# opensensor/thingino-accel

Measured on AMD Instinct MI355X. Metric: images/sec yolov5s_int8 640x640 batch256, higher is better.
Workload: dtype int8

## Files before the change

thingino-accel_amd/csrc/hip/conv_i8.hip:

```cpp
#include "conv_i8_common.hpp"

#ifndef I8M_ABL
#define I8M_ABL 0
#endif
template <int BPX, int BN, int STAGES, int KS = 1, int NW = 4>
__global__ __launch_bounds__(NW * 64) void conv_i8_mfma(const mhip_conv_i8_t p, const long total_pix, const int k64,
                                                         const int8_t *__restrict__ zeros, const unsigned noc,
                                                         const unsigned nblk, const int lg_inc, const unsigned kw_magic,
                                                         const fastdiv_t dhw, const fastdiv_t dow, const int bufmode,
                                                         const unsigned in_bytes) {
    ANAT_BEGIN();
    const bool POW2 = lg_inc >= 0;
    const bool masked = p.kh * p.kw <= 32;
    constexpr int SLICE = (BPX + BN) * BK;
    constexpr int STAGE = KS * SLICE;
    constexpr int NWN = BN == 128 ? 2 : 1;
    constexpr int NWM = NW / NWN;
    constexpr int WPX = BPX / NWM / 16;
    constexpr int WOC = BN / NWN / 16;
    constexpr int XROWS = BPX / NW;
    constexpr int XI = XROWS / 16;
    constexpr int LW = (BN / 16 + NW - 1) / NW;
    constexpr int L = XI + LW;
    static_assert(XI >= 1 && XROWS % 16 == 0, "every wave fetches whole 16-row pieces of the pixel tile");
    extern __shared__ __attribute__((aligned(16))) int8_t dynlds[];
    uint8_t *slut = (uint8_t *)dynlds;
    lds_base_must_be_zero(dynlds);
    long *rowoff = (long *)(dynlds + LUTB);
    int8_t *lds = dynlds + BPX * 8 + LUTB;

    const int tid = threadIdx.x, lane = tid & 63;
    const int wv = __builtin_amdgcn_readfirstlane(tid >> 6);
    const unsigned id = xcd_remap(blockIdx.x, nblk);
    const long pix0 = (long)(id / noc) * BPX;
    const int oc0 = (int)(id % noc) * BN;
    const int hw = p.out_h * p.out_w;

    const int wm = wv % NWM, wn = wv / NWM;
    const int pxw = wm * (WPX * 16), ocw = wn * (WOC * 16);
    v4i acc[WOC][WPX];
    init_acc<WPX, WOC>(p, acc, oc0 + ocw);
    if (p.lut2) { if (tid < 128) ((uint32_t *)slut)[tid] = ((const uint32_t *)p.lut2)[tid]; }
    else if (p.lut && tid < 64) ((uint32_t *)slut)[tid] = ((const uint32_t *)p.lut)[tid];
    fill_rowoff<BPX>(p, rowoff, [=](int row) { long q = pix0 + row; return q < total_pix ? q : -1L; }, (unsigned)hw, dhw);

    const int schunk = (lane & 3) ^ (((lane >> 4) & 1) << 1);
    const int8_t *xwin[XI];
    unsigned tapmask[XI];
    int iy0[XI], ix0[XI];
#pragma unroll
    for (int j = 0; j < XI; j++) {
        const long pix = pix0 + wv * XROWS + j * 16 + (lane >> 2);
        const bool valid = pix < total_pix;
        const unsigned f = valid ? fdiv((unsigned)pix, dhw) : 0u;
        const unsigned rem = valid ? (unsigned)pix - f * (unsigned)hw : 0u;
        const int oy = (int)fdiv(rem, dow), ox = (int)(rem - (unsigned)oy * (unsigned)p.out_w);
        iy0[j] = valid ? oy * p.stride_h - p.pad_top : -(1 << 28);
        ix0[j] = ox * p.stride_w - p.pad_left;
        xwin[j] = p.in + (size_t)f * p.in_stride + ((long)iy0[j] * p.in_w + ix0[j]) * p.in_c;
        unsigned m = 0;
        if (masked) {
            const int kx_lo = ix0[j] < 0 ? -ix0[j] : 0, kx_hi = p.in_w - ix0[j] < p.kw ? p.in_w - ix0[j] : p.kw;
            const unsigned colbits = kx_hi > kx_lo ? ((kx_hi >= 32 ? ~0u : (1u << kx_hi) - 1u) & ~((1u << kx_lo) - 1u)) : 0u;
            for (int r = 0; r < p.kh; r++) {
                const int iy = iy0[j] + r;
                if (iy >= 0 && iy < p.in_h) m |= colbits << (r * p.kw);
            }
        }
        tapmask[j] = m;
    }
    const int8_t *wsrc[LW];
    int wq[LW];
#pragma unroll
    for (int j = 0; j < LW; j++) {
        wq[j] = BN / 16 >= NW ? wv * LW + j : (wv % (BN / 16));
        wsrc[j] = p.w + (size_t)(oc0 + wq[j] * 16 + (lane >> 2)) * k64 + schunk * 16;
    }
    const __amdgpu_buffer_rsrc_t xrs = __builtin_amdgcn_make_buffer_rsrc((void *)p.in, 0, (int)in_bytes, 0x00020000);
    const __amdgpu_buffer_rsrc_t wrs = __builtin_amdgcn_make_buffer_rsrc((void *)p.w, 0, p.oc_pad * k64, 0x00020000);
    int xvoff[XI], wvoff[LW];
    if (bufmode) {
#pragma unroll
        for (int j = 0; j < XI; j++) xvoff[j] = (int)(xwin[j] - p.in) + schunk * 16;
#pragma unroll
        for (int j = 0; j < LW; j++) wvoff[j] = (oc0 + wq[j] * 16 + (lane >> 2)) * k64 + schunk * 16;
    }
    int ky = 0, kx = 0, rc = schunk * 16;
    if (!POW2) {
        while (rc >= p.in_c) { rc -= p.in_c; kx++; }
        while (kx >= p.kw) { kx -= p.kw; ky++; }
    }
    const int taps = p.kh * p.kw;

    const int nks = k64 / BK;
    auto issue = [&](int ks, int stage) {
        int8_t *sb = lds + stage * STAGE + (KS > 1 ? (ks % KS) * SLICE : 0);
        if (bufmode) {
            const int utap = (ks * BK) >> lg_inc, urc = (ks * BK) & ((1 << lg_inc) - 1);
            const int uky = (int)(((unsigned)utap * kw_magic) >> 16), ukx = utap - uky * p.kw;
            const int ukoff = (uky * p.in_w + ukx) * p.in_c + urc;
            const bool uvalid = utap < taps;
#pragma unroll
            for (int j = 0; j < XI; j++) {
                const bool ok = uvalid & (((tapmask[j] >> utap) & 1u) != 0u);
                if (!(I8M_ABL & 8)) blds16(xrs, ok ? xvoff[j] + ukoff : -1, 0, sb + (wv * XROWS + j * 16) * BK);
            }
#pragma unroll
            for (int j = 0; j < LW; j++)
                if (!(I8M_ABL & 8)) blds16(wrs, wvoff[j], ks * BK, sb + BPX * BK + wq[j] * 16 * BK);
            return;
        }
        bool kvalid;
        if (POW2) {
            const unsigned pos = (unsigned)(ks * BK + schunk * 16);
            const unsigned tap = pos >> lg_inc;
            rc = (int)(pos & ((1u << lg_inc) - 1u));
            ky = (int)((tap * kw_magic) >> 16);
            kx = (int)tap - ky * p.kw;
            kvalid = (int)tap < taps;
        } else {
            kvalid = ky < p.kh;
        }
        const long koff = ((long)ky * p.in_w + kx) * p.in_c + rc;
        const int tap = ky * p.kw + kx;
#pragma unroll
        for (int j = 0; j < XI; j++) {
            bool ok;
            if (masked) {
                ok = kvalid & ((tapmask[j] >> tap) & 1u);
            } else {
                const int iy = iy0[j] + ky, ix = ix0[j] + kx;
                ok = kvalid & (iy >= 0) & (iy < p.in_h) & (ix >= 0) & (ix < p.in_w);
            }
            const int8_t *src = ok ? xwin[j] + koff : zeros;
            glds16(src, sb + (wv * XROWS + j * 16) * BK);
        }
#pragma unroll
        for (int j = 0; j < LW; j++) glds16(wsrc[j] + ks * BK, sb + BPX * BK + wq[j] * 16 * BK);
        if (!POW2) {
            rc += BK;
            while (rc >= p.in_c) { rc -= p.in_c; kx++; }
            while (kx >= p.kw) { kx -= p.kw; ky++; }
        }
    };

    const int nst = I8M_ABL & 2 ? 0 : nks / KS;
#pragma unroll
    for (int s = 0; s < STAGES - 1; s++)
        if (s < nst)
#pragma unroll
            for (int u = 0; u < KS; u++) issue(s * KS + u, s);

    const int frow = lane & 15, fchunk = lane >> 4;
    int stage = 0, nstage = STAGES - 1;
    ANAT_NOW(1);
    for (int st = 0; st < nst; st++) {
        const int ahead = nst - 1 - st;
        if (STAGES >= 4 && ahead >= 2) wait_vmcnt<2 * L * KS>();
        else if (STAGES >= 3 && ahead >= 1) wait_vmcnt<L * KS>();
        else wait_vmcnt<0>();
        __builtin_amdgcn_s_barrier();
        asm volatile("" ::: "memory");
#pragma unroll
        for (int u = 0; u < KS; u++) {
            const int8_t *xs = lds + stage * STAGE + u * SLICE, *ws = xs + BPX * BK;
            v4i xb[WPX], wa[WOC];
#pragma unroll
            for (int t = 0; t < WPX; t++) xb[t] = *(const v4i *)(xs + lds_off(pxw + t * 16 + frow, fchunk));
#pragma unroll
            for (int s = 0; s < WOC; s++) wa[s] = *(const v4i *)(ws + lds_off(ocw + s * 16 + frow, fchunk));
            if (u == 0 && st + STAGES - 1 < nst)
#pragma unroll
                for (int v = 0; v < KS; v++) issue((st + STAGES - 1) * KS + v, nstage);
#pragma unroll
            for (int s = 0; s < WOC; s++)
#pragma unroll
                for (int t = 0; t < WPX; t++) {
                    if (I8M_ABL & 4) asm volatile("" ::"v"(wa[s]), "v"(xb[t]));
                    else acc[s][t] = __builtin_amdgcn_mfma_i32_16x16x64_i8(wa[s], xb[t], acc[s][t], 0, 0, 0);
                }
        }
        stage = stage + 1 == STAGES ? 0 : stage + 1;
        nstage = nstage + 1 == STAGES ? 0 : nstage + 1;
    }
    ANAT_NOW(2);
    __syncthreads();
    if (I8M_ABL & 1) {
        int fold = 0;
#pragma unroll
        for (int s = 0; s < WOC; s++)
#pragma unroll
            for (int t = 0; t < WPX; t++) fold ^= acc[s][t][0] ^ acc[s][t][1] ^ acc[s][t][2] ^ acc[s][t][3];
        if (fold == 0x12345678) p.out[0] = 1;
        return;
    }
    epilogue<BPX, BN, WPX, WOC, true>(p, acc, lds, slut, rowoff, oc0, pxw, ocw, hw);
    ANAT_END(p);
}

__device__ __forceinline__ int lds_off128(int row, int chunk8) { return row * 128 + ((chunk8 ^ ((row >> 1) & 7)) << 4); }
template <int BPX, int BN, int NW>
__global__ __launch_bounds__(NW * 64) void conv_i8_r128(const mhip_conv_i8_t p, const long total_pix, const int k128,
                                                         const unsigned noc, const unsigned nblk, const int lg_inc,
                                                         const unsigned kw_magic, const fastdiv_t dhw, const fastdiv_t dow,
                                                         const unsigned in_bytes) {
    constexpr int STAGE = (BPX + BN) * 128;
    constexpr int NWN = BN == 128 ? 2 : 1;
    constexpr int NWM = NW / NWN;
    constexpr int WPX = BPX / NWM / 16;
    constexpr int WOC = BN / NWN / 16;
    constexpr int XI = BPX / 8 / NW;
    constexpr int WI = BN / 8 / NW;
    static_assert(XI >= 1 && WI >= 1 && BPX % (8 * NW) == 0 && BN % (8 * NW) == 0, "whole 8-row pieces per wave");
    extern __shared__ __attribute__((aligned(16))) int8_t dynlds[];
    uint8_t *slut = (uint8_t *)dynlds;
    lds_base_must_be_zero(dynlds);
    long *rowoff = (long *)(dynlds + LUTB);
    int8_t *lds = dynlds + BPX * 8 + LUTB;

    const int tid = threadIdx.x, lane = tid & 63;
    const int wv = __builtin_amdgcn_readfirstlane(tid >> 6);
    const unsigned id = xcd_remap(blockIdx.x, nblk);
    const long pix0 = (long)(id / noc) * BPX;
    const int oc0 = (int)(id % noc) * BN;
    const int hw = p.out_h * p.out_w;
    const int wm = wv % NWM, wn = wv / NWM;
    const int pxw = wm * (WPX * 16), ocw = wn * (WOC * 16);
    v4i acc[WOC][WPX];
    init_acc<WPX, WOC>(p, acc, oc0 + ocw);
    if (p.lut2) { if (tid < 128) ((uint32_t *)slut)[tid] = ((const uint32_t *)p.lut2)[tid]; }
    else if (p.lut && tid < 64) ((uint32_t *)slut)[tid] = ((const uint32_t *)p.lut)[tid];
    fill_rowoff<BPX>(p, rowoff, [=](int row) { long q = pix0 + row; return q < total_pix ? q : -1L; }, (unsigned)hw, dhw);

    const int lrow = lane >> 3, lslot = lane & 7;
    int xvoff[XI];
    unsigned tapmask[XI];
#pragma unroll
    for (int j = 0; j < XI; j++) {
        const int trow = (wv * XI + j) * 8 + lrow;
        const long pix = pix0 + trow;
        const bool valid = pix < total_pix;
        const unsigned f = valid ? fdiv((unsigned)pix, dhw) : 0u;
        const unsigned rem = valid ? (unsigned)pix - f * (unsigned)hw : 0u;
        const int oy = (int)fdiv(rem, dow), ox = (int)(rem - (unsigned)oy * (unsigned)p.out_w);
        const int iy0 = oy * p.stride_h - p.pad_top, ix0 = ox * p.stride_w - p.pad_left;
        const int chunk = lslot ^ ((trow >> 1) & 7);
        xvoff[j] = (int)(f * (unsigned)p.in_stride) + (iy0 * p.in_w + ix0) * p.in_c + chunk * 16;
        const int kx_lo = ix0 < 0 ? -ix0 : 0, kx_hi = p.in_w - ix0 < p.kw ? p.in_w - ix0 : p.kw;
        const unsigned colbits = kx_hi > kx_lo ? ((kx_hi >= 32 ? ~0u : (1u << kx_hi) - 1u) & ~((1u << kx_lo) - 1u)) : 0u;
        unsigned m = 0;
        for (int r = 0; r < p.kh; r++) {
            const int iy = iy0 + r;
            if (iy >= 0 && iy < p.in_h) m |= colbits << (r * p.kw);
        }
        tapmask[j] = valid ? m : 0u;
    }
    int wvoff[WI];
#pragma unroll
    for (int j = 0; j < WI; j++) {
        const int trow = (wv * WI + j) * 8 + lrow;
        wvoff[j] = (oc0 + trow) * k128 + (lslot ^ ((trow >> 1) & 7)) * 16;
    }
    const __amdgpu_buffer_rsrc_t xrs = __builtin_amdgcn_make_buffer_rsrc((void *)p.in, 0, (int)in_bytes, 0x00020000);
    const __amdgpu_buffer_rsrc_t wrs = __builtin_amdgcn_make_buffer_rsrc((void *)p.w, 0, p.oc_pad * k128, 0x00020000);
    const int taps = p.kh * p.kw;
    const int nst = k128 / 128;
    auto issue = [&](int st, int buf) {
        int8_t *sb = lds + buf * STAGE;
        const int utap = (st * 128) >> lg_inc, urc = (st * 128) & ((1 << lg_inc) - 1);
        const int uky = (int)(((unsigned)utap * kw_magic) >> 16), ukx = utap - uky * p.kw;
        const int ukoff = (uky * p.in_w + ukx) * p.in_c + urc;
        const bool uvalid = utap < taps;
#pragma unroll
        for (int j = 0; j < XI; j++) {
            const bool ok = uvalid & (((tapmask[j] >> utap) & 1u) != 0u);
            blds16(xrs, ok ? xvoff[j] + ukoff : -1, 0, sb + (wv * XI + j) * 1024);
// ... 416 lines not shown
    v4i acc[WOC][WPX];
    init_acc<WPX, WOC>(p, acc, oc0);

    load_global(0);
    store_lds(0);
    __syncthreads();
    const int frow = lane & 15, fchunk = lane >> 4;
    const int pxw = wv * 32;
    for (int ks = 0; ks < nks; ks++) {
        const int buf = ks & 1;
        if (ks + 1 < nks) load_global(ks + 1);
        v4i xb[WPX];
#pragma unroll
        for (int t = 0; t < WPX; t++) xb[t] = *(const v4i *)(lds + buf * STAGE + lds_off(pxw + t * 16 + frow, fchunk));
#pragma unroll
        for (int s = 0; s < WOC; s++) {
            v4i wa = *(const v4i *)(lds + buf * STAGE + BP * BK + lds_off(s * 16 + frow, fchunk));
#pragma unroll
            for (int t = 0; t < WPX; t++) acc[s][t] = __builtin_amdgcn_mfma_i32_16x16x64_i8(wa, xb[t], acc[s][t], 0, 0, 0);
        }
        if (ks + 1 < nks) store_lds(buf ^ 1);
        __syncthreads();
    }
    epilogue<BP, BN, WPX, WOC>(p, acc, lds, slut, rowoff, oc0, pxw, 0, hw);
}

extern "C" int mhip_conv_i8_oc_row(int oc, int oc_pad) {
    const int G = (oc_pad % 64 == 0) ? 64 : 32, NS = G / 16;
    const int g = oc / G, local = oc - g * G;
    const int q = local / (4 * NS), rem = local - q * 4 * NS, s = rem >> 2, r = rem & 3;
    return g * G + s * 16 + q * 4 + r;
}

extern "C" int mhip_conv_i8_is_safe(float cs) {
    return cs == cs && cs < 0.99f && cs > -0.99f;
}

extern "C" int mhip_conv_i8_lut2_ok(float cs) {
    if (!mhip_conv_i8_is_safe(cs)) return 0;
    const float a = cs < 0 ? -cs : cs;
    if (!(a >= 1e-6f)) return 0;
    const float quirk = 0.49999997f;
    const double a0 = (double)quirk / (double)a;
    for (int d = -3; d <= 3; d++) {
        const double c = (double)(long long)(a0 + 0.5) + d;
        if (c < 1.0 || c > 2147483647.0) continue;
        volatile float prod = (float)(int)c * a;
        if (prod == quirk) return 0;
    }
    return 1;
}

extern "C" int mhip_conv_i8_small_c(int in_c, int kw, int out_c) { return in_c <= 4 && kw <= 8 && out_c <= 64; }

extern "C" void mhip_conv_i8_pack_geom(int in_c, int kw, int out_c, int *row_pad, int *oc_pad, int *c_eff) {
    const int small = mhip_conv_i8_small_c(in_c, kw, out_c);
    if (row_pad) *row_pad = small ? 32 : (kw * in_c + 15) & ~15;
    if (oc_pad) *oc_pad = (out_c + 31) & ~31;
    if (c_eff) *c_eff = small ? 4 : in_c;
}

static tune_t g_tune;
static int env_int(const char *name, int dflt) {
    const char *e = getenv(name);
    return e ? atoi(e) : dflt;
}
const tune_t &conv_i8_tune_state() {
    if (!g_tune.init) {
        g_tune.persist = env_int("MARS_HIP_PERSIST", 1);
        g_tune.persist_stages = env_int("MARS_HIP_PSTAGES", 2);
        g_tune.persist_maxk = env_int("MARS_HIP_PERSIST_MAXK", 8);
        g_tune.persist_slots = env_int("MARS_HIP_PSLOTS", 0);
        g_tune.stages = env_int("MARS_HIP_STAGES", 0);
        g_tune.bpx = env_int("MARS_HIP_BPX", 0);
        g_tune.variant = env_int("MARS_HIP_VARIANT", 0);
        g_tune.bufmode = env_int("MARS_HIP_BUFMODE", 1);
        g_tune.wres = env_int("MARS_HIP_WRES", 3);
        g_tune.rgb_direct = env_int("MARS_HIP_RGB_DIRECT", 1);
        g_tune.small_batch = env_int("MARS_HIP_SMALL_BATCH", 1);
        g_tune.rows = env_int("MARS_HIP_ROWS", 1);
        g_tune.few_wgs = env_int("MARS_HIP_FEW_WGS", 256);
        g_tune.patch_ring = env_int("MARS_HIP_PATCH_RING", 0);
        g_tune.patch_lds_kb = env_int("MARS_HIP_PATCH_LDS_KB", 80);
        g_tune.init = 1;
    }
    return g_tune;
}
static inline const tune_t &tune() { return conv_i8_tune_state(); }
static int tune_access(const char *key, int value, int *get) {
    (void)conv_i8_tune_state();
    struct { const char *k; int *v; } tab[] = {{"persist", &g_tune.persist}, {"persist_stages", &g_tune.persist_stages},
                                               {"persist_maxk", &g_tune.persist_maxk}, {"persist_slots", &g_tune.persist_slots}, {"wres", &g_tune.wres}, {"rgb_direct", &g_tune.rgb_direct}, {"small_batch", &g_tune.small_batch},
                                               {"rows", &g_tune.rows}, {"few_wgs", &g_tune.few_wgs}, {"patch_ring", &g_tune.patch_ring}, {"patch_lds_kb", &g_tune.patch_lds_kb}, {"stages", &g_tune.stages}, {"bpx", &g_tune.bpx}, {"variant", &g_tune.variant}, {"bufmode", &g_tune.bufmode}};
    for (auto &e : tab)
        if (key && !strcmp(key, e.k)) {
            if (get) *get = *e.v;
            else *e.v = value;
            return 0;
        }
    return -1;
}
extern "C" int mhip_conv_i8_tune(const char *key, int value) { return tune_access(key, value, nullptr); }
extern "C" int mhip_conv_i8_tune_get(const char *key, int *value) { return value ? tune_access(key, 0, value) : -1; }

static int buf_mode(const mhip_conv_i8_t *p, int k64) {
    if (!tune().bufmode) return 0;
    return p->in_c >= 64 && (p->in_c & (p->in_c - 1)) == 0 && p->kh * p->kw <= 32 && (long)p->kh * p->kw * (p->kw - 1) < 65536 &&
           in_extent_bytes(p) <= 0x7fffffffL && (long)p->oc_pad * k64 <= 0x7fffffffL;
}

template <int BPX, int BN, int STAGES, int KS = 1, int NW = 4>
static int launch_mfma(const mhip_conv_i8_t *p, long total_pix, int k64) {
    const unsigned npt = (unsigned)((total_pix + BPX - 1) / BPX), noc = (unsigned)(p->oc_pad / BN);
    const unsigned nblk = npt * noc;
    const int nks = k64 / BK, nst = nks / KS, used = nst < STAGES ? nst : STAGES;
    if (KS > 1 && (nks % KS) != 0) return -1;
    size_t ring = (size_t)used * KS * (BPX + BN) * BK, tile = (size_t)BPX * (BN + OPAD);
    const size_t lds = BPX * 8 + LUTB + (ring > tile ? ring : tile);
    if (lds > 64 * 1024) {
        static bool attr = false;
        if (!attr && hipFuncSetAttribute((const void *)conv_i8_mfma<BPX, BN, STAGES, KS, NW>, hipFuncAttributeMaxDynamicSharedMemorySize,
                                         (int)(BPX * 8 + LUTB + (size_t)STAGES * KS * (BPX + BN) * BK)) != hipSuccess)
            return mhip_check(hipErrorUnknown, "conv_i8_mfma LDS attribute");
        attr = true;
    }
    int lg = -1;
    if ((p->in_c & (p->in_c - 1)) == 0 && (long)p->kh * p->kw * (p->kw - 1) < 65536) {
        lg = 0;
        while ((1 << lg) < p->in_c) lg++;
    }
    const unsigned magic = ((65536u + (unsigned)p->kw - 1u) / (unsigned)p->kw);
    hipLaunchKernelGGL((conv_i8_mfma<BPX, BN, STAGES, KS, NW>), dim3(nblk), dim3(NW * 64), lds, mhip_stream_native(), *p, total_pix,
                       k64, (const int8_t *)mhip_zero_page(), noc, nblk, lg, magic,
                       make_fastdiv((unsigned)(p->out_h * p->out_w)), make_fastdiv((unsigned)p->out_w),
                       lg >= 0 ? buf_mode(p, k64) : 0, (unsigned)in_extent_bytes(p));
    return mhip_check(hipGetLastError(), "conv_i8_mfma launch");
}


template <int BPX, int BN>
static size_t wres_lds(int k64) { return LUTB + 2 * (size_t)BPX * BK + (size_t)(k64 / BK) * BN * BK; }

template <int BPX, int BN, int STAGES, bool HAS_LUT, bool SEG = false, bool PAIR = false>
static int launch_persist_t(const mhip_conv_i8_t *p, long total_pix, int k64, int lg, unsigned magic,
                            const mhip_conv_i8_t *second = nullptr, int wres = 0) {
    if (BN == 16 && (p->out_c > 16 || p->oc_pad != 32 || (PAIR && (second->out_c > 16 || second->oc_pad != 32)))) return -1;
    const unsigned noc0 = BN == 16 ? 1u : (unsigned)(p->oc_pad / BN);
    const unsigned npt = (unsigned)((total_pix + BPX - 1) / BPX), noc = noc0 + (PAIR ? (BN == 16 ? 1u : (unsigned)(second->oc_pad / BN)) : 0u);
    conv_out_side_t alt;
    memset(&alt, 0, sizeof(alt));
    if (PAIR) {
        alt.out = second->out; alt.out_stride = second->out_stride; alt.w = second->w; alt.bias = second->bias;
        alt.lut = second->lut; alt.lut2 = second->lut2; alt.out_c = second->out_c; alt.relu = second->relu; alt.out_pix_stride = second->out_pix_stride;
        alt.out_ch_off = second->out_ch_off; alt.cs = second->cs;
    }
    if (PAIR) alt.out_bytes = (unsigned)persist_out_bytes(second);
    if (wres && STAGES != 2) return -1;
    const size_t lds = wres ? wres_lds<BPX, BN>(k64) : LUTB + (size_t)STAGES * (BPX + BN) * BK;
    if (wres) {
        static bool attr = false;
        if (!attr && hipFuncSetAttribute((const void *)conv_i8_persist<BPX, BN, STAGES, HAS_LUT, SEG, PAIR>,
                                         hipFuncAttributeMaxDynamicSharedMemorySize, 80 * 1024) != hipSuccess)
            return mhip_check(hipErrorUnknown, "conv_i8_persist LDS attribute");
        attr = true;
        int occ = 0, dev = 0;
        hipDeviceProp_t prop;
        if (hipOccupancyMaxActiveBlocksPerMultiprocessor(&occ, conv_i8_persist<BPX, BN, STAGES, HAS_LUT, SEG, PAIR>, NTHREADS, lds) != hipSuccess ||
            hipGetDevice(&dev) != hipSuccess || hipGetDeviceProperties(&prop, dev) != hipSuccess)
            return mhip_check(hipErrorUnknown, "conv_i8_persist occupancy query");
        unsigned g = (unsigned)((occ > 0 ? occ : 1) * prop.multiProcessorCount) / noc;
        if (tune().persist_slots > 0) g = (unsigned)tune().persist_slots / noc;
        if (g < 1) g = 1;
        if (g > npt) g = npt;
        hipLaunchKernelGGL((conv_i8_persist<BPX, BN, STAGES, HAS_LUT, SEG, PAIR>), dim3(noc * g), dim3(NTHREADS), lds,
                           mhip_stream_native(), *p, (unsigned)total_pix, k64, (const int8_t *)mhip_zero_page(), noc, npt, g, lg,
                           magic, make_fastdiv((unsigned)(p->out_h * p->out_w)), make_fastdiv((unsigned)p->out_w),
                           (unsigned)persist_out_bytes(p), alt, noc0, SEG ? 0 : buf_mode(p, k64), (unsigned)in_extent_bytes(p), 1);
        return mhip_check(hipGetLastError(), "conv_i8_persist (resident weights) launch");
    }
    static int slots = 0;
    if (!slots) {
        int occ = 0, dev = 0;
        hipDeviceProp_t prop;
        if (hipOccupancyMaxActiveBlocksPerMultiprocessor(&occ, conv_i8_persist<BPX, BN, STAGES, HAS_LUT, SEG, PAIR>, NTHREADS, lds) != hipSuccess ||
            hipGetDevice(&dev) != hipSuccess || hipGetDeviceProperties(&prop, dev) != hipSuccess)
            return mhip_check(hipErrorUnknown, "conv_i8_persist occupancy query");
        slots = (occ > 0 ? occ : 1) * prop.multiProcessorCount;
    }
    unsigned ngrp = (unsigned)(tune().persist_slots > 0 ? tune().persist_slots : 4 * slots) / noc;
    if (ngrp < 1) ngrp = 1;
    if (ngrp > npt) ngrp = npt;
    hipLaunchKernelGGL((conv_i8_persist<BPX, BN, STAGES, HAS_LUT, SEG, PAIR>), dim3(noc * ngrp), dim3(NTHREADS), lds,
                       mhip_stream_native(), *p, (unsigned)total_pix, k64, (const int8_t *)mhip_zero_page(), noc, npt, ngrp, lg,
                       magic, make_fastdiv((unsigned)(p->out_h * p->out_w)), make_fastdiv((unsigned)p->out_w),
                       (unsigned)persist_out_bytes(p), alt, noc0, SEG ? 0 : buf_mode(p, k64), (unsigned)in_extent_bytes(p), 0);
    return mhip_check(hipGetLastError(), "conv_i8_persist launch");
}

#define NVARIANTS 20
struct variant_t {
    int persist, bpx, stages, patch, ks2, w8, wres, r128, rows;
};
static int variant_code(const variant_t &v) {
    if (v.rows) return 20;
    if (v.r128) return 17 + v.r128;
    if (v.wres) return v.bpx == 256 ? 15 : 14;
    if (v.w8) return 13;
    if (v.ks2) return 12;
    if (v.patch) return v.patch == 16 ? 10 : (v.patch == 8 ? 9 : 11);
    return 1 + (v.persist ? 1 : 0) + (v.bpx == 256 ? 2 : 0) + (v.stages == 3 ? 4 : 0);
}
static variant_t variant_of(int code) {
    if (code == 20) return variant_t{0, 0, 0, 0, 0, 0, 0, 0, 1};
    if (code == 18 || code == 19) return variant_t{0, 0, 0, 0, 0, 0, 0, code - 17, 0};
    if (code == 14 || code == 15) return variant_t{1, code == 15 ? 256 : 128, 2, 0, 0, 0, 1, 0, 0};
    if (code == 13) return variant_t{0, 256, 3, 0, 0, 1, 0, 0, 0};
    if (code == 12) return variant_t{0, 128, 2, 0, 1, 0, 0, 0, 0};
    if (code >= 9 && code <= 11) return variant_t{0, 0, 0, code == 10 ? 16 : (code == 9 ? 8 : 4), 0, 0, 0, 0, 0};
// ... 352 lines not shown
```

thingino-accel_amd/csrc/hip/conv_i8_common.hpp:

```cpp
#pragma once
#include <hip/hip_runtime.h>
#include <stdint.h>
#include <stdlib.h>
#include <string.h>
#include <type_traits>

#include "../mhip.h"

extern "C" hipStream_t mhip_stream_native(void);
extern "C" int mhip_check(hipError_t e, const char *what);
extern "C" const void *mhip_zero_page(void);

typedef int v4i __attribute__((ext_vector_type(4)));
typedef int v2i __attribute__((ext_vector_type(2)));

#ifdef ANATOMY
struct anat_rec_t {
    unsigned key, wg, hwid, xcc;
    unsigned long long t[4];
};
static __device__ anat_rec_t *g_anat_buf;
static __device__ unsigned g_anat_cap;
#define ANAT_SETTER(NAME)                                                                                                    \
    extern "C" int NAME(void *buf, unsigned cap) {                                                                          \
// ... 281 lines not shown
        }
        if (DIRECT) {
            const long off = rowoff[prow];
            if (off >= 0 && oc0 + chan < p.out_c) {
                int8_t *d = p.out + off + oc0 + chan;
                if (WOC == 4) *(v4i *)d = (v4i){(int)pk[0], (int)pk[1], (int)pk[2], (int)pk[3]};
                else if (WOC == 2) *(uint2 *)d = make_uint2(pk[0], pk[WOC > 1 ? 1 : 0]);
                else *(uint32_t *)d = pk[0];
            }
        } else {
#pragma unroll
            for (int s = 0; s < WOC; s++) *(uint32_t *)(tile + prow * ROW + chan + s * 4) = pk[s];
        }
    }
    if (DIRECT) return;
    __syncthreads();
    const int ncols = p.out_c - oc0 < BN ? p.out_c - oc0 : BN;
    if (!p.out_nchw && ((p.out_c | p.out_pix_stride | p.out_ch_off) & 15) == 0) {
        constexpr int CPR = BN / 16;
        for (int id = tid; id < BPX * CPR; id += (int)blockDim.x) {
            const int row = id / CPR, c = id - row * CPR;
            const long off = rowoff[row];
            if (off < 0 || c * 16 >= ncols) continue;
            const int8_t *s = tile + row * ROW + c * 16;
            v4i v = {*(const int *)s, *(const int *)(s + 4), *(const int *)(s + 8), *(const int *)(s + 12)};
            *(v4i *)(p.out + off + oc0 + c * 16) = v;
        }
    } else if (!p.out_nchw) {
        constexpr int CPR = BN / 16;
        for (int id = tid; id < BPX * CPR; id += (int)blockDim.x) {
            const int row = id / CPR, c = id - row * CPR;
            const long off = rowoff[row];
            if (off < 0 || c * 16 >= ncols) continue;
            const int8_t *s = tile + row * ROW + c * 16;
            int8_t *d = p.out + off + oc0 + c * 16;
            if (c * 16 + 16 <= ncols) {
                v4i v = {*(const int *)s, *(const int *)(s + 4), *(const int *)(s + 8), *(const int *)(s + 12)};
                __builtin_memcpy(d, &v, 16);
            } else {
                const int rem = ncols - c * 16;
                int o = 0;
                if (rem & 8) { __builtin_memcpy(d, s, 8); o = 8; }
                if (rem & 4) { __builtin_memcpy(d + o, s + o, 4); o += 4; }
                if (rem & 2) { __builtin_memcpy(d + o, s + o, 2); o += 2; }
                if (rem & 1) d[o] = s[o];
            }
        }
    } else {
        for (int id = tid; id < BPX * BN; id += (int)blockDim.x) {
            const int c = id / BPX, row = id - c * BPX;
            const long off = rowoff[row];
            if (off < 0 || c >= ncols) continue;
            p.out[off + (size_t)(oc0 + c) * hw] = tile[row * ROW + c];
        }
    }
}

template <int BPX, int BN, int WPX, int WOC, bool LUT0 = false>
__device__ __forceinline__ void epilogue(const mhip_conv_i8_t &p, v4i (&acc)[WOC][WPX], int8_t *tile, const uint8_t *slut,
                                         const long *rowoff, int oc0, int pxw, int ocw, int hw) {
    const bool direct = !p.out_nchw && ((p.out_c | p.out_pix_stride | p.out_ch_off) & 15) == 0;
#define EPI(L, S, D) epilogue_t<BPX, BN, WPX, WOC, L, S, D, LUT0>(p, acc, tile, slut, rowoff, oc0, pxw, ocw, hw)
    if (direct) {
        if (p.lut) { if (p.safe) EPI(true, true, true); else EPI(true, false, true); }
        else { if (p.safe) EPI(false, true, true); else EPI(false, false, true); }
    } else {
        if (p.lut) { if (p.safe) EPI(true, true, false); else EPI(true, false, false); }
        else { if (p.safe) EPI(false, true, false); else EPI(false, false, false); }
    }
#undef EPI
}

template <int WPX, int WOC>
__device__ __forceinline__ void init_acc(const mhip_conv_i8_t &p, v4i (&acc)[WOC][WPX], int ocbase) {
    const int lane = threadIdx.x & 63;
#pragma unroll
    for (int s = 0; s < WOC; s++) {
        const v4i b = p.bias ? *(const v4i *)(p.bias + ocbase + s * 16 + (lane >> 4) * 4) : (v4i){0, 0, 0, 0};
#pragma unroll
        for (int t = 0; t < WPX; t++) acc[s][t] = b;
    }
}


struct tune_t {
    int init;
    int persist;
    int persist_stages;
    int persist_maxk;
    int persist_slots;
    int stages;
    int bpx;
    int variant;
    int bufmode;
    int small_batch;
    int rgb_direct;
    int wres;
    int few_wgs;
    int rows;
    int patch_ring;
    int patch_lds_kb;
};
const tune_t &conv_i8_tune_state();

extern "C" int mhip_conv_i8_small_c(int in_c, int kw, int out_c);

static inline long in_extent_bytes(const mhip_conv_i8_t *p) {
    return (long)(p->frames - 1) * (long)p->in_stride + (long)p->in_h * p->in_w * p->in_c;
}
static inline long persist_out_bytes(const mhip_conv_i8_t *p) {
    const long pstride = p->out_pix_stride ? p->out_pix_stride : p->out_c;
    return (long)(p->frames - 1) * (long)p->out_stride + (long)p->out_h * p->out_w * pstride;
}
static inline bool conv_i8_direct_rows(const mhip_conv_i8_t *p) {
    return !p->out_nchw && ((p->out_c | p->out_pix_stride | p->out_ch_off) & 15) == 0;
}

bool conv_i8_patch_ok(const mhip_conv_i8_t *p, int th, int *ring);
int conv_i8_launch_patch(const mhip_conv_i8_t *p, int k64, int th);
int conv_i8_pre_tile_rows(const mhip_conv_i8_t *p);
bool conv_i8_rows_ok(const mhip_conv_i8_t *p);
int conv_i8_launch_rows(const mhip_conv_i8_t *p);
int conv_i8_try_rgb(const mhip_conv_i8_t *p, int k64);
int conv_i8_try_smallc(const mhip_conv_i8_t *p, int k64);
```

thingino-accel_amd/csrc/hip/mhip_runtime.hip:

```cpp
#include <hip/hip_runtime.h>
#include <stdio.h>
#include <stdlib.h>
#include <string.h>

#include "../mhip.h"

static hipStream_t g_stream = nullptr;
static hipStream_t g_aux = nullptr;
static hipStream_t g_up = nullptr;
static hipStream_t g_down = nullptr;
static hipStream_t g_seconds[3] = {nullptr, nullptr, nullptr};
static int g_use_aux = 0;
static int g_ready = 0;
static int g_device = -1;
static char g_err[256] = "";
static void *g_zero_page = nullptr;

static hipStream_t stream_of(int which) {
    if (which == 1) return g_aux;
    if (which == 2 || which == 3) {
        hipStream_t &st = which == 2 ? g_up : g_down;
        if (!st && hipStreamCreateWithFlags(&st, hipStreamNonBlocking) != hipSuccess) st = nullptr;
        return st ? st : g_stream;
    }
    if (which >= 4 && which <= 6) {
        hipStream_t &st = g_seconds[which - 4];
        if (!st) {
            int lo = 0, hi = 0;
            if (hipDeviceGetStreamPriorityRange(&lo, &hi) != hipSuccess) lo = hi = 0;
            if (hipStreamCreateWithPriority(&st, hipStreamNonBlocking, hi) != hipSuccess) st = nullptr;
        }
        return st ? st : g_stream;
    }
    return g_stream;
}
extern "C" hipStream_t mhip_stream_native(void) { return stream_of(g_use_aux); }

extern "C" int mhip_check(hipError_t e, const char *what) {
    if (e == hipSuccess) return 0;
    snprintf(g_err, sizeof(g_err), "%s: %s", what, hipGetErrorString(e));
    if (getenv("MARS_VERBOSE")) fprintf(stderr, "mars-hip: %s\n", g_err);
    return -(int)e;
}

extern "C" const char *mhip_last_error(void) { return g_err; }

extern "C" int mhip_init(int device_hint) {
    if (g_ready) return 0;
    int n = 0;
    if (hipGetDeviceCount(&n) != hipSuccess || n <= 0) {
        snprintf(g_err, sizeof(g_err), "no HIP device visible");
        return -1;
    }
    if (device_hint >= n) {
        snprintf(g_err, sizeof(g_err), "device %d requested, %d visible", device_hint, n);
        return -1;
    }
    int dev = device_hint >= 0 ? device_hint : 0;
    hipDeviceProp_t prop;
    if (mhip_check(hipGetDeviceProperties(&prop, dev), "hipGetDeviceProperties")) return -1;
    if (strncmp(prop.gcnArchName, "gfx950", 6) != 0) {
        snprintf(g_err, sizeof(g_err), "device %d is %s, this build targets gfx950 (MI355X)", dev, prop.gcnArchName);
        return -2;
    }
    if (mhip_check(hipSetDevice(dev), "hipSetDevice")) return -1;
    int prio_lo = 0, prio_hi = 0;
    if (hipDeviceGetStreamPriorityRange(&prio_lo, &prio_hi) != hipSuccess) prio_lo = prio_hi = 0;
    if (mhip_check(hipStreamCreateWithPriority(&g_stream, hipStreamNonBlocking, prio_hi), "hipStreamCreate")) return -3;
    if (mhip_check(hipStreamCreateWithPriority(&g_aux, hipStreamNonBlocking, prio_lo), "hipStreamCreate aux")) return -3;
    if (mhip_check(hipMalloc(&g_zero_page, 256), "hipMalloc zero page") ||
        mhip_check(hipMemset(g_zero_page, 0, 256), "hipMemset zero page"))
        return -3;
    g_device = dev;
    g_ready = 1;
    return 0;
}

extern "C" void mhip_tail_release(void);
extern "C" void mhip_shutdown(void) {
    if (!g_ready) return;
    (void)hipStreamSynchronize(g_stream);
    (void)hipStreamSynchronize(g_aux);
    mhip_tail_release();
    (void)hipStreamDestroy(g_stream);
    (void)hipStreamDestroy(g_aux);
    if (g_up) { (void)hipStreamSynchronize(g_up); (void)hipStreamDestroy(g_up); }
    if (g_down) { (void)hipStreamSynchronize(g_down); (void)hipStreamDestroy(g_down); }
    for (int k = 0; k < 3; k++) {
        if (g_seconds[k]) { (void)hipStreamSynchronize(g_seconds[k]); (void)hipStreamDestroy(g_seconds[k]); }
        g_seconds[k] = nullptr;
    }
    g_up = g_down = nullptr;
    g_aux = nullptr;
    g_use_aux = 0;
    if (g_zero_page) (void)hipFree(g_zero_page);
    g_zero_page = nullptr;
    g_stream = nullptr;
    g_ready = 0;
}

extern "C" int mhip_ready(void) { return g_ready; }
extern "C" const void *mhip_zero_page(void) { return g_zero_page; }

extern "C" int mhip_device_info(int *cu_count, int *lds_bytes, int *gfx_version, size_t *hbm_bytes) {
    if (!g_ready) return -1;
    hipDeviceProp_t prop;
    if (mhip_check(hipGetDeviceProperties(&prop, g_device), "hipGetDeviceProperties")) return -1;
    if (cu_count) *cu_count = prop.multiProcessorCount;
    if (lds_bytes) *lds_bytes = (int)prop.maxSharedMemoryPerMultiProcessor;
    if (gfx_version) *gfx_version = atoi(prop.gcnArchName + 3);
    if (hbm_bytes) *hbm_bytes = prop.totalGlobalMem;
    return 0;
}

extern "C" void *mhip_stream(void) { return (void *)g_stream; }

extern "C" int mhip_sync(void) {
    int rc = mhip_check(hipStreamSynchronize(g_stream), "hipStreamSynchronize");
    int rc2 = mhip_check(hipStreamSynchronize(g_aux), "hipStreamSynchronize aux");
    if (g_up && mhip_check(hipStreamSynchronize(g_up), "hipStreamSynchronize upload") && !rc) rc = -1;
    if (g_down && mhip_check(hipStreamSynchronize(g_down), "hipStreamSynchronize download") && !rc) rc = -1;
    for (int k = 0; k < 3; k++)
        if (g_seconds[k] && mhip_check(hipStreamSynchronize(g_seconds[k]), "hipStreamSynchronize second") && !rc) rc = -1;
    return rc ? rc : rc2;
}
extern "C" void mhip_select_aux(int on) { g_use_aux = on ? 1 : 0; }
extern "C" void mhip_select_stream(int which) { g_use_aux = which >= 0 && which <= 6 ? which : 0; }
extern "C" int mhip_stream_wait(int which, void *ev) {
    return mhip_check(hipStreamWaitEvent(stream_of(which), (hipEvent_t)ev, 0), "hipStreamWaitEvent");
}
extern "C" int mhip_event_sync(void *ev) { return mhip_check(hipEventSynchronize((hipEvent_t)ev), "hipEventSynchronize"); }

extern "C" void *mhip_malloc(size_t bytes) {
    void *p = nullptr;
    if (!g_ready) return nullptr;
    if (mhip_check(hipMalloc(&p, bytes ? bytes : 256), "hipMalloc")) return nullptr;
    return p;
}

extern "C" void mhip_free(void *p) {
    if (p) (void)hipFree(p);
}

extern "C" void *mhip_host_alloc(size_t bytes) {
    void *p = nullptr;
    if (!g_ready) return nullptr;
    if (mhip_check(hipHostMalloc(&p, bytes ? bytes : 256, hipHostMallocDefault), "hipHostMalloc")) return nullptr;
    return p;
}

extern "C" void mhip_host_free(void *p) {
    if (p) (void)hipHostFree(p);
}

extern "C" int mhip_memset_async(void *dst, int value, size_t bytes) {
    return mhip_check(hipMemsetAsync(dst, value, bytes, mhip_stream_native()), "hipMemsetAsync");
}
extern "C" int mhip_h2d_async(void *dst, const void *src, size_t bytes) {
    return mhip_check(hipMemcpyAsync(dst, src, bytes, hipMemcpyHostToDevice, mhip_stream_native()), "H2D");
}
extern "C" int mhip_d2h_async(void *dst, const void *src, size_t bytes) {
    return mhip_check(hipMemcpyAsync(dst, src, bytes, hipMemcpyDeviceToHost, mhip_stream_native()), "D2H");
}
extern "C" int mhip_d2d_async(void *dst, const void *src, size_t bytes) {
    return mhip_check(hipMemcpyAsync(dst, src, bytes, hipMemcpyDeviceToDevice, mhip_stream_native()), "D2D");
}
// ... 53 lines not shown
```

Baseline: 56790.

## Add split-K for tail tiles of int8 MFMA conv with slab combine

Adds an optional split-K mode where tiles in the last partial wave are divided along K into pieces. Each piece writes partial accumulators to a global slab, and the last arriving piece sums them and runs the epilogue. This targets wave-quantization idle time at the grid tail, paid for with slab traffic, atomics and workspace allocation. It also adds amdgpu_waves_per_eu hints to the kernel, which apply unconditionally, while split-K defaults off through MARS_HIP_SPLIT=0.

```diff
diff --git a/thingino-accel_amd/csrc/hip/conv_i8.hip b/thingino-accel_amd/csrc/hip/conv_i8.hip
--- a/thingino-accel_amd/csrc/hip/conv_i8.hip
+++ b/thingino-accel_amd/csrc/hip/conv_i8.hip
@@ -4,11 +4,12 @@
 #define I8M_ABL 0
 #endif
 template <int BPX, int BN, int STAGES, int KS = 1, int NW = 4>
-__global__ __launch_bounds__(NW * 64) void conv_i8_mfma(const mhip_conv_i8_t p, const long total_pix, const int k64,
+__global__ __launch_bounds__(NW * 64) __attribute__((amdgpu_waves_per_eu(NW == 8 ? 4 : (BPX * BN >= 256 * 128 ? 2 : 1)))) void conv_i8_mfma(const mhip_conv_i8_t p, const long total_pix, const int k64,
                                                          const int8_t *__restrict__ zeros, const unsigned noc,
                                                          const unsigned nblk, const int lg_inc, const unsigned kw_magic,
                                                          const fastdiv_t dhw, const fastdiv_t dow, const int bufmode,
-                                                         const unsigned in_bytes) {
+                                                         const unsigned in_bytes, const unsigned nfull, const int split,
+                                                         int *__restrict__ slabs, unsigned *__restrict__ arrivals) {
     ANAT_BEGIN();
     const bool POW2 = lg_inc >= 0;
     const bool masked = p.kh * p.kw <= 32;
@@ -31,7 +32,9 @@
 
     const int tid = threadIdx.x, lane = tid & 63;
     const int wv = __builtin_amdgcn_readfirstlane(tid >> 6);
-    const unsigned id = xcd_remap(blockIdx.x, nblk);
+    const bool ispiece = blockIdx.x >= nfull;
+    const unsigned jp = blockIdx.x - nfull, id = ispiece ? nfull + jp / (unsigned)split : xcd_remap(blockIdx.x, nfull);
+    const int piece = ispiece ? (int)(jp % (unsigned)split) : 0;
     const long pix0 = (long)(id / noc) * BPX;
     const int oc0 = (int)(id % noc) * BN;
     const int hw = p.out_h * p.out_w;
@@ -40,6 +43,7 @@
     const int pxw = wm * (WPX * 16), ocw = wn * (WOC * 16);
     v4i acc[WOC][WPX];
     init_acc<WPX, WOC>(p, acc, oc0 + ocw);
+    if (piece) zero_acc<WPX, WOC>(acc);
     if (p.lut2) { if (tid < 128) ((uint32_t *)slut)[tid] = ((const uint32_t *)p.lut2)[tid]; }
     else if (p.lut && tid < 64) ((uint32_t *)slut)[tid] = ((const uint32_t *)p.lut)[tid];
     fill_rowoff<BPX>(p, rowoff, [=](int row) { long q = pix0 + row; return q < total_pix ? q : -1L; }, (unsigned)hw, dhw);
@@ -93,7 +97,10 @@
     const int taps = p.kh * p.kw;
 
     const int nks = k64 / BK;
-    auto issue = [&](int ks, int stage) {
+    const int nst_all = I8M_ABL & 2 ? 0 : nks / KS;
+    const int sbeg = ispiece ? piece * nst_all / split : 0, send = ispiece ? (piece + 1) * nst_all / split : nst_all;
+    auto issue = [&](int ksr, int stage) {
+        const int ks = ksr + sbeg * KS;
         int8_t *sb = lds + stage * STAGE + (KS > 1 ? (ks % KS) * SLICE : 0);
         if (bufmode) {
             const int utap = (ks * BK) >> lg_inc, urc = (ks * BK) & ((1 << lg_inc) - 1);
@@ -144,7 +151,7 @@
         }
     };
 
-    const int nst = I8M_ABL & 2 ? 0 : nks / KS;
+    const int nst = send - sbeg;
 #pragma unroll
     for (int s = 0; s < STAGES - 1; s++)
         if (s < nst)
@@ -192,6 +199,11 @@
 #pragma unroll
             for (int t = 0; t < WPX; t++) fold ^= acc[s][t][0] ^ acc[s][t][1] ^ acc[s][t][2] ^ acc[s][t][3];
         if (fold == 0x12345678) p.out[0] = 1;
+        return;
+    }
+    if (ispiece && !split_combine<WPX, WOC, NW * 64>(acc, slabs + (size_t)(id - nfull) * split * (WOC * WPX * NW * 256), arrivals + (id - nfull),
+                                                     piece, split, (unsigned *)lds)) {
+        ANAT_END(p);
         return;
     }
     epilogue<BPX, BN, WPX, WOC, true>(p, acc, lds, slut, rowoff, oc0, pxw, ocw, hw);
@@ -774,6 +786,9 @@
         g_tune.few_wgs = env_int("MARS_HIP_FEW_WGS", 256);
         g_tune.patch_ring = env_int("MARS_HIP_PATCH_RING", 0);
         g_tune.patch_lds_kb = env_int("MARS_HIP_PATCH_LDS_KB", 80);
+        g_tune.split = env_int("MARS_HIP_SPLIT", 0);
+        g_tune.split_s = env_int("MARS_HIP_SPLIT_S", 0);
+        g_tune.split_slots = env_int("MARS_HIP_SPLIT_SLOTS", 0);
         g_tune.init = 1;
     }
     return g_tune;
@@ -783,7 +798,8 @@
     (void)conv_i8_tune_state();
     struct { const char *k; int *v; } tab[] = {{"persist", &g_tune.persist}, {"persist_stages", &g_tune.persist_stages},
                                                {"persist_maxk", &g_tune.persist_maxk}, {"persist_slots", &g_tune.persist_slots}, {"wres", &g_tune.wres}, {"rgb_direct", &g_tune.rgb_direct}, {"small_batch", &g_tune.small_batch},
-                                               {"rows", &g_tune.rows}, {"few_wgs", &g_tune.few_wgs}, {"patch_ring", &g_tune.patch_ring}, {"patch_lds_kb", &g_tune.patch_lds_kb}, {"stages", &g_tune.stages}, {"bpx", &g_tune.bpx}, {"variant", &g_tune.variant}, {"bufmode", &g_tune.bufmode}};
+                                               {"rows", &g_tune.rows}, {"few_wgs", &g_tune.few_wgs}, {"patch_ring", &g_tune.patch_ring}, {"patch_lds_kb", &g_tune.patch_lds_kb}, {"stages", &g_tune.stages}, {"bpx", &g_tune.bpx}, {"variant", &g_tune.variant}, {"bufmode", &g_tune.bufmode},
+                                               {"split", &g_tune.split}, {"split_s", &g_tune.split_s}, {"split_slots", &g_tune.split_slots}};
     for (auto &e : tab)
         if (key && !strcmp(key, e.k)) {
             if (get) *get = *e.v;
@@ -799,6 +815,68 @@
     if (!tune().bufmode) return 0;
     return p->in_c >= 64 && (p->in_c & (p->in_c - 1)) == 0 && p->kh * p->kw <= 32 && (long)p->kh * p->kw * (p->kw - 1) < 65536 &&
            in_extent_bytes(p) <= 0x7fffffffL && (long)p->oc_pad * k64 <= 0x7fffffffL;
+}
+
+#define SPLIT_SLAB_BYTES (64u << 20)
+#define SPLIT_MAX_TILES 4096u
+extern "C" int mhip_conv_i8_split_plan(unsigned nblk, unsigned slots, int nst, unsigned slab_bytes, int mode, int force_s,
+                                       unsigned *nfull) {
+    *nfull = nblk;
+    if (mode <= 0 || slots == 0 || nst < 2 || slab_bytes == 0) return 1;
+    const unsigned tail = nblk % slots;
+    if (tail == 0 || (nblk < slots && mode < 2)) return 1;
+    if (tail > SPLIT_MAX_TILES) return 1;
+    const double PRO = 3.0, EPI = 4.0, SLAB = 1.0, READ = 1.5;
+    const double whole = nst + PRO + EPI;
+    int best = 1;
+    double best_cost = mode >= 2 ? 1e30 : whole;
+    const int smax = nst < 8 ? nst : 8;
+    for (int s = 2; s <= smax; s++) {
+        if ((unsigned long long)tail * s * slab_bytes > SPLIT_SLAB_BYTES) break;
+        if (force_s && s != force_s) continue;
+        const double rounds = (double)(((unsigned long long)tail * s + slots - 1) / slots);
+        const double cost = rounds * ((double)nst / s + PRO + SLAB) + (s - 1) * READ + EPI;
+        if (cost < best_cost) best_cost = cost, best = s;
+    }
+    if (best > 1) *nfull = nblk - tail;
+    return best;
+}
+
+struct split_ws_t {
+    hipStream_t st;
+    int *slabs;
+    unsigned *arrivals;
+};
+static split_ws_t g_split_ws[8];
+static const split_ws_t *split_workspace(hipStream_t st) {
+    for (auto &w : g_split_ws)
+        if (w.slabs && w.st == st) return &w;
+    hipStreamCaptureStatus cap = hipStreamCaptureStatusNone;
+    if (hipStreamIsCapturing(st, &cap) != hipSuccess || cap != hipStreamCaptureStatusNone) return nullptr;
+    for (auto &w : g_split_ws)
+        if (!w.slabs) {
+            void *a = nullptr, *b = nullptr;
+            if (hipMalloc(&a, SPLIT_SLAB_BYTES) != hipSuccess) return nullptr;
+            if (hipMalloc(&b, SPLIT_MAX_TILES * sizeof(unsigned)) != hipSuccess ||
+                hipMemsetAsync(b, 0, SPLIT_MAX_TILES * sizeof(unsigned), st) != hipSuccess) {
+                (void)hipFree(a);
+                if (b) (void)hipFree(b);
+                return nullptr;
+            }
+            w.st = st;
+            w.slabs = (int *)a;
+            w.arrivals = (unsigned *)b;
+            return &w;
+        }
+    return nullptr;
+}
+
+extern "C" void mhip_conv_i8_split_release(void) {
+    for (auto &w : g_split_ws) {
+        if (w.slabs) (void)hipFree(w.slabs);
+        if (w.arrivals) (void)hipFree(w.arrivals);
+        w = split_ws_t{};
+    }
 }
 
 template <int BPX, int BN, int STAGES, int KS = 1, int NW = 4>
@@ -822,10 +900,29 @@
         while ((1 << lg) < p->in_c) lg++;
     }
     const unsigned magic = ((65536u + (unsigned)p->kw - 1u) / (unsigned)p->kw);
-    hipLaunchKernelGGL((conv_i8_mfma<BPX, BN, STAGES, KS, NW>), dim3(nblk), dim3(NW * 64), lds, mhip_stream_native(), *p, total_pix,
+    unsigned nfull = nblk;
+    int split = 1;
+    const split_ws_t *ws = nullptr;
+    if (tune().split && lg >= 0) {
+        static unsigned slots = 0;
+        if (!slots) {
+            int occ = 0, dev = 0;
+            hipDeviceProp_t prop;
+            if (hipOccupancyMaxActiveBlocksPerMultiprocessor(&occ, conv_i8_mfma<BPX, BN, STAGES, KS, NW>, NW * 64, lds) != hipSuccess ||
+                hipGetDevice(&dev) != hipSuccess || hipGetDeviceProperties(&prop, dev) != hipSuccess)
+                return mhip_check(hipErrorUnknown, "conv_i8_mfma occupancy query");
+            slots = (unsigned)((occ > 0 ? occ : 1) * prop.multiProcessorCount);
+        }
+        split = mhip_conv_i8_split_plan(nblk, tune().split_slots > 0 ? (unsigned)tune().split_slots : slots, nst,
+                                        (unsigned)BPX * BN * 4, tune().split, tune().split_s, &nfull);
+        if (split > 1 && !(ws = split_workspace(mhip_stream_native()))) split = 1, nfull = nblk;
+    }
+    const unsigned grid = nfull + (nblk - nfull) * (unsigned)split;
+    hipLaunchKernelGGL((conv_i8_mfma<BPX, BN, STAGES, KS, NW>), dim3(grid), dim3(NW * 64), lds, mhip_stream_native(), *p, total_pix,
                        k64, (const int8_t *)mhip_zero_page(), noc, nblk, lg, magic,
                        make_fastdiv((unsigned)(p->out_h * p->out_w)), make_fastdiv((unsigned)p->out_w),
-                       lg >= 0 ? buf_mode(p, k64) : 0, (unsigned)in_extent_bytes(p));
+                       lg >= 0 ? buf_mode(p, k64) : 0, (unsigned)in_extent_bytes(p), nfull, split,
+                       ws ? ws->slabs : nullptr, ws ? ws->arrivals : nullptr);
     return mhip_check(hipGetLastError(), "conv_i8_mfma launch");
 }
 
diff --git a/thingino-accel_amd/csrc/hip/conv_i8_common.hpp b/thingino-accel_amd/csrc/hip/conv_i8_common.hpp
--- a/thingino-accel_amd/csrc/hip/conv_i8_common.hpp
+++ b/thingino-accel_amd/csrc/hip/conv_i8_common.hpp
@@ -387,6 +387,49 @@
     }
 }
 
+template <int WPX, int WOC>
+__device__ __forceinline__ void zero_acc(v4i (&acc)[WOC][WPX]) {
+#pragma unroll
+    for (int s = 0; s < WOC; s++)
+#pragma unroll
+        for (int t = 0; t < WPX; t++) acc[s][t] = (v4i){0, 0, 0, 0};
+}
+
+template <int WPX, int WOC, int NT>
+__device__ __forceinline__ bool split_combine(v4i (&acc)[WOC][WPX], int *tile_slabs, unsigned *arrival, int piece, int split,
+                                              unsigned *flag) {
+    constexpr int NV = WOC * WPX;
+    const int tid = threadIdx.x;
+    const __amdgpu_buffer_rsrc_t rs = __builtin_amdgcn_make_buffer_rsrc(tile_slabs, 0, split * NV * NT * 16, 0x00020000);
+    constexpr int SC1 = 16;
+#pragma unroll
+    for (int s = 0; s < WOC; s++)
+#pragma unroll
+        for (int t = 0; t < WPX; t++)
+            __builtin_amdgcn_raw_buffer_store_b128(acc[s][t], rs, ((piece * NV + s * WPX + t) * NT + tid) * 16, 0, SC1);
+    asm volatile("s_waitcnt vmcnt(0)" ::: "memory");
+    __syncthreads();
+    if (tid == 0) flag[0] = __hip_atomic_fetch_add(arrival, 1u, __ATOMIC_RELAXED, __HIP_MEMORY_SCOPE_AGENT);
+    __syncthreads();
+    if (flag[0] != (unsigned)(split - 1)) return false;
+    if (tid == 0) __hip_atomic_store(arrival, 0u, __ATOMIC_RELAXED, __HIP_MEMORY_SCOPE_AGENT);
+    for (int q = 0; q < split; q++) {
+        if (q == piece) continue;
+        v4i part[WOC][WPX];
+#pragma unroll
+        for (int s = 0; s < WOC; s++)
+#pragma unroll
+            for (int t = 0; t < WPX; t++)
+                part[s][t] = __builtin_bit_cast(v4i, __builtin_amdgcn_raw_buffer_load_b128(rs, ((q * NV + s * WPX + t) * NT + tid) * 16, 0, SC1));
+#pragma unroll
+        for (int s = 0; s < WOC; s++)
+#pragma unroll
+            for (int t = 0; t < WPX; t++) acc[s][t] += part[s][t];
+    }
+    __syncthreads();
+    return true;
+}
+
 
 struct tune_t {
     int init;
@@ -405,6 +448,9 @@
     int rows;
     int patch_ring;
     int patch_lds_kb;
+    int split;
+    int split_s;
+    int split_slots;
 };
 const tune_t &conv_i8_tune_state();
 
diff --git a/thingino-accel_amd/csrc/hip/mhip_runtime.hip b/thingino-accel_amd/csrc/hip/mhip_runtime.hip
--- a/thingino-accel_amd/csrc/hip/mhip_runtime.hip
+++ b/thingino-accel_amd/csrc/hip/mhip_runtime.hip
@@ -77,11 +77,15 @@
 }
 
 extern "C" void mhip_tail_release(void);
+extern "C" void mhip_conv_i8_split_release(void);
 extern "C" void mhip_shutdown(void) {
     if (!g_ready) return;
     (void)hipStreamSynchronize(g_stream);
     (void)hipStreamSynchronize(g_aux);
+    for (int k = 0; k < 3; k++)
+        if (g_seconds[k]) (void)hipStreamSynchronize(g_seconds[k]);
     mhip_tail_release();
+    mhip_conv_i8_split_release();
     (void)hipStreamDestroy(g_stream);
     (void)hipStreamDestroy(g_aux);
     if (g_up) { (void)hipStreamSynchronize(g_up); (void)hipStreamDestroy(g_up); }
```

Measured after the change: 56700, median of 3. No clear change (-0.1%).
